# zkp-gravity/0g-halo2

Measured on AMD Instinct MI355X. Metric: create_proof proofs/hour, model_28input_256entry_1hash_1bpi, higher is better.
Workload: dtype u32x8 (254-bit Montgomery integers)

## Files before the change

### 0g-halo2_amd/csrc/common.h

```cpp
#pragma once

#include <hip/hip_runtime.h>
#include <hip/hip_ext.h>

#include <array>
#include <atomic>
#include <cstdarg>
#include <cstdio>
#include <cstring>
#include <map>
#include <mutex>
#include <string>
#include <vector>

#include "../../include/zg_halo2.h"
#include "curve.h"

namespace zg {

void set_error(const char* fmt, ...);

#define ZG_HIP(call)                                                                         \
    do {                                                                                     \
        hipError_t _e = (call);                                                              \
// ... 16 lines not shown

#define ZG_REQUIRE(cond, status, ...)   \
    do {                                \
        if (!(cond)) {                  \
            ::zg::set_error(__VA_ARGS__); \
            return (status);            \
        }                               \
    } while (0)

static_assert(sizeof(Fe) == 32 && sizeof(zg_fr) == 32, "field element layout");
static_assert(sizeof(Affine) == 64 && sizeof(zg_g1_affine) == 64, "affine layout");
static_assert(sizeof(Jac) == 96 && sizeof(zg_g1) == 96, "jacobian layout");
static_assert(sizeof(XYZZ) == 128, "xyzz layout");

struct WsBlock {
    void* p = nullptr;
    size_t cap = 0;
    bool used = false;
};

struct TwiddleKey {
    uint32_t log_n;
    std::array<uint64_t, 4> omega;
    bool operator<(const TwiddleKey& o) const {
        if (log_n != o.log_n) return log_n < o.log_n;
        return omega < o.omega;
    }
};

}

namespace zg {
struct DeviceState {
    std::mutex mu;
    std::map<TwiddleKey, Fe*> twiddles;
    int refs = 0;
    bool msm_attrs = false, ntt_attrs = false;
};
DeviceState& device_state(int device);
}

struct zg_ctx {
    int device = 0;
    hipStream_t stream = nullptr;
    int num_cus = 256;
    std::vector<zg::WsBlock> pool;
    void* pinned = nullptr;
    size_t pinned_cap = 0;
    std::recursive_mutex mu;
// ... 60 lines not shown
            failed = true;
            return nullptr;
        }
        held.push_back(p);
        return reinterpret_cast<T*>(p);
    }
};
int pinned_reserve(zg_ctx* ctx, size_t bytes);
void gate_yield(zg_ctx* ctx);
uint32_t tuning_generation();

zg_ctx::ProfRec* prof_slot(zg_ctx* ctx, const char* name, double algo_bytes, double unit_bytes);
#define ZG_LAUNCH_U(ctx, name, bytes, unit, kernel, grid, block, lds, ...)                               \
    do {                                                                                                 \
        zg_ctx::ProfRec* _zg_r = (ctx)->profiling ? ::zg::prof_slot((ctx), (name), (double)(bytes), (double)(unit)) : nullptr; \
        if (_zg_r)                                                                                       \
            hipExtLaunchKernelGGL(kernel, grid, block, lds, (ctx)->stream, _zg_r->e0, _zg_r->e1, 0, __VA_ARGS__); \
        else                                                                                             \
            hipLaunchKernelGGL(kernel, grid, block, lds, (ctx)->stream, __VA_ARGS__);                    \
    } while (0)
#define ZG_LAUNCH(ctx, name, bytes, kernel, grid, block, lds, ...) \
    ZG_LAUNCH_U(ctx, name, bytes, 0.0, kernel, grid, block, lds, __VA_ARGS__)

int get_twiddles(zg_ctx* ctx, uint32_t log_n, const Fe& omega, Fe** out);

Fe host_domain_omega(uint32_t log_n);

enum Knob : int {
    K_MSM_C,
    K_MSM_K,
    K_MSM_K_LAT,
    K_MSM_RB,
    K_MSM_LANES,
    K_MSM_STRIP,
    K_MSM_NAF,
    K_MSM_NAF_GL,
    K_MSM_RUNS,
    K_EVALH_GROUPED,
    K_EVALH9,
    K_SPLIT_DOMAIN,
    K_LAT_SPLIT_K,
    K_LAT_FULL_C,
    K_LAT_FULL_K,
    K_LAZY_DOT,
    K_MSM_AFFINE,
    K_MSM_HEAVY,
    K_LAT_PULL,
// ... 11 lines not shown
```

### 0g-halo2_amd/csrc/field9.h

```cpp
#pragma once

#include "curve.h"
#include "field.h"

namespace zg {

struct F9 {
    int32_t l[9];
};

constexpr int32_t MASK29 = (1 << 29) - 1;

struct Fq9Params {
    static __device__ __forceinline__ int32_t p(int i) {
        constexpr int32_t P[9] = {0x187cfd47, 0x010460b6, 0x1c72a34f, 0x02d522d0, 0x1585d978,
                                  0x02db40c0, 0x00a6e141, 0x0e5c2634, 0x0030644e};
        return P[i];
    }
    static constexpr uint32_t INV29 = 0x04866389u;
    static __device__ __forceinline__ F9 one() {
        return F9{{0x157ccc21, 0x141c2758, 0x185230d3, 0x014c0419, 0x0aa36fb9, 0x1d4240ce, 0x11d54c07, 0x052ac7a8, 0x000dc836}};
    }
    static __device__ __forceinline__ F9 k256() {
        return F9{{0x058f0d9d, 0x1aea1c6e, 0x11c2cf74, 0x11d651eb, 0x1462c0a7, 0x11b7bc3c, 0x1cbd99ba, 0x183340fb, 0x000e0a77}};
// ... 363 lines not shown
            inf = true;
            return;
        }
        const F9 u = f9_norm(f9_add(qy, qy));
        const F9 v = Fq9::sqr(u);
        const F9 w = Fq9::mul(u, v);
        const F9 s = Fq9::mul(qx, v);
        const F9 x2 = Fq9::sqr(qx);
        const F9 m = f9_norm(f9_add(f9_add(x2, x2), x2));
        a.x = f9_norm(f9_sub(f9_sub(Fq9::sqr(m), s), s));
        a.y = f9_norm(f9_sub(Fq9::mul(m, f9_norm(f9_sub(s, a.x))), Fq9::mul(w, f9_norm(qy))));
        a.zz = v;
        a.zzz = w;
        return;
    }
    const F9 ppp = Fq9::mul(p, pp);
    const F9 qq = Fq9::mul(a.x, pp);
    const F9 x3 = f9_norm(f9_sub(f9_sub(f9_sub(Fq9::sqr(r), ppp), qq), qq));
    const F9 t = f9_sub(qq, x3);
    a.y = Fq9::mul2<true>(r, t, a.y, ppp);
    a.x = x3;
    a.zz = Fq9::mul(a.zz, pp);
    a.zzz = Fq9::mul(a.zzz, ppp);
}

__device__ __noinline__ XYZZ9 xyzz9_dbl(const XYZZ9& a) {
    if (xyzz9_is_identity(a)) return a;
    XYZZ9 o;
    const F9 u = f9_norm(f9_add(a.y, a.y));
    const F9 v = Fq9::sqr(u);
    const F9 w = Fq9::mul(u, v);
    const F9 s = Fq9::mul(a.x, v);
    const F9 xx = Fq9::sqr(a.x);
    const F9 m = f9_norm(f9_add(f9_add(xx, xx), xx));
    o.x = f9_norm(f9_sub(f9_sub(Fq9::sqr(m), s), s));
    o.y = f9_norm(f9_sub(Fq9::mul(m, f9_norm(f9_sub(s, o.x))), Fq9::mul(w, a.y)));
    o.zz = Fq9::mul(v, a.zz);
    o.zzz = Fq9::mul(w, a.zzz);
    return o;
}

__device__ __forceinline__ XYZZ9 xyzz9_add(const XYZZ9& a, const XYZZ9& b) {
    if (xyzz9_is_identity(a)) return b;
    if (xyzz9_is_identity(b)) return a;
    const F9 u1 = Fq9::mul(a.x, b.zz);
    const F9 u2 = Fq9::mul(b.x, a.zz);
// ... 254 lines not shown
```

### 0g-halo2_amd/csrc/msm.hip

```cpp
#include <cstdlib>

#include "msm.h"
#include "field9.h"

namespace zg {

constexpr uint32_t MSM_K_THROUGHPUT = 48, MSM_K_LATENCY = 16;
constexpr uint32_t MSM_MAX_C = 16;
constexpr uint32_t MSM_LEN_BINS = 128;
constexpr uint32_t MSM_HEAVY = 16;
constexpr uint32_t MSM_HEAVY_THROUGHPUT = 4;
constexpr uint32_t MSM_AFFINE_ROUNDS = 0;
constexpr uint32_t MSM_MAX_BATCH = 4096;

__device__ __forceinline__ Fe ld_fe_g(const Fe* p) {
    Fe r;
    const uint4* q = reinterpret_cast<const uint4*>(p);
    uint4 a = q[0], b = q[1];
    r.l[0] = a.x; r.l[1] = a.y; r.l[2] = a.z; r.l[3] = a.w;
    r.l[4] = b.x; r.l[5] = b.y; r.l[6] = b.z; r.l[7] = b.w;
    return r;
}
__device__ __forceinline__ void st_fe_g(Fe* p, const Fe& v) {
    uint4* q = reinterpret_cast<uint4*>(p);
// ... 567 lines not shown
        }
    };
    scan(true);
    const F9 before = t ? sh[t - 1] : Fq9Params::one();
    if (t == AFF_TOP - 1) {
        const Fe inv8 = Fq::inv(f9_reduce_pack<Fq9Params>(sh[t]));
        tinv = Fq9::mul(f9_unpack(inv8), Fq9Params::k271());
    }
    __syncthreads();
    scan(false);
    const F9 after = t + 1 < AFF_TOP ? sh[t + 1] : Fq9Params::one();
    F9 u = Fq9::mul(Fq9::mul(tinv, before), after);
    if (t >= n2) return;
    size_t e = t + ((n2 - 1 - t) / AFF_TOP) * AFF_TOP;
#pragma unroll 1
    for (;; e -= AFF_TOP) {
        const F9 v = ld_f9_soa(val2, n2, e);
        st_f9_soa(val2, n2, e, Fq9::mul(u, ld_f9_soa(pfx2, n2, e)));
        u = Fq9::mul(u, v);
        if (e < AFF_TOP) break;
    }
}

template <bool PAIR, bool AFF = false>
__global__ __launch_bounds__(256) void msm_accumulate_kernel(
    const Affine* __restrict__ table_a, const Affine* __restrict__ table_b, uint32_t split, uint32_t n_table,
    uint32_t c, uint32_t windows, uint32_t n,
    const uint32_t* __restrict__ tot, const uint32_t* __restrict__ toff, const uint32_t* __restrict__ ttotal,
    const uint32_t* __restrict__ sorted, uint32_t max_tasks, XYZZ9* __restrict__ partial,
    const Affine* __restrict__ run_a, const Affine* __restrict__ run_b, uint64_t run_mask, uint32_t per,
    const uint32_t* __restrict__ stoff, const uint32_t* __restrict__ sbucket, size_t cap, uint32_t R,
    const Affine* __restrict__ pts) {
    const uint32_t lane = blockIdx.x * blockDim.x + threadIdx.x;
    const uint32_t t = PAIR ? lane >> 1 : lane;
    const bool role_a = !PAIR || (lane & 1u) == 0;
    uint32_t b = blockIdx.y;
    if (t >= ttotal[b]) return;
    const uint32_t vj = b % per;
    const bool runs = vj < 64 && ((run_mask >> vj) & 1ull);
    const Affine* table = vj < split ? (runs ? run_a : table_a) : (runs ? run_b : table_b);
    const uint32_t nb = 1u << (c - 1);
    const uint32_t* to = toff + (size_t)b * (nb + 2);
    const uint32_t* sto = stoff + (size_t)b * (nb + 2);
    uint32_t lo = 0, hi = nb + 1;
    while (hi - lo > 1) {
        uint32_t mid = (lo + hi) >> 1;
        if (sto[mid] <= t) lo = mid;
        else hi = mid;
    }
    const uint32_t k = sbucket[(size_t)b * (nb + 1) + lo];
    const uint32_t j = t - sto[lo];
    const uint32_t first = tot[(size_t)b * (nb + 2) + k] >> R;
    const uint32_t total = (tot[(size_t)b * (nb + 2) + k + 1] >> R) - first;
    const uint32_t nt = to[k + 1] - to[k];
    const uint32_t share = total / nt, extra = total % nt;
    const uint32_t start = first + j * share + (j < extra ? j : extra);
    const uint32_t len = share + (j < extra ? 1u : 0u);
    const uint32_t* so = sorted + (size_t)b * cap + start;
    XYZZ9* dst = partial + (size_t)b * max_tasks + to[k] + j;
    bool inf = true;
    if constexpr (PAIR) {
        PairAcc acc;
        for (uint32_t e = 0; e < len; e++) {
            uint32_t ent = so[e];
            uint32_t i = ent & 0x7fffffu, w = (ent >> 23) & 0xffu;
            const Affine* src = table + (size_t)w * n_table + i;
            const F9 qx = f9_unpack(ld_fe_g(&src->x));
            F9 qy = f9_unpack(ld_fe_g(&src->y));
            if (f9_limbs_zero(qx) && f9_limbs_zero(qy)) continue;
            if (ent >> 31) qy = f9_neg(qy);
            xmadd_pair(acc, inf, qx, qy, role_a);
        }
        if (inf) {
            if (role_a) st_xyzz9(dst, xyzz9_identity());
        } else if (role_a) {
            st_f9(&dst->x, acc.m);
            st_f9(&dst->zz, acc.z);
        } else {
            st_f9(&dst->y, acc.m);
            st_f9(&dst->zzz, acc.z);
        }
    } else if constexpr (AFF) {
        XYZZ9 acc;
        const Affine* src = pts + (size_t)b * (cap >> R) + start;
        for (uint32_t e = 0; e < len; e++) {
            const F9 qx = f9_unpack(ld_fe_g(&src[e].x));
            const F9 qy = f9_unpack(ld_fe_g(&src[e].y));
            if (f9_limbs_zero(qx) && f9_limbs_zero(qy)) continue;
            xyzz9_madd(acc, inf, qx, qy);
        }
        st_xyzz9(dst, inf ? xyzz9_identity() : acc);
    } else {
        XYZZ9 acc;
        for (uint32_t e = 0; e < len; e++) {
            uint32_t ent = so[e];
            uint32_t i = ent & 0x7fffffu, w = (ent >> 23) & 0xffu;
            const Affine* src = table + (size_t)w * n_table + i;
            const F9 qx = f9_unpack(ld_fe_g(&src->x));
            F9 qy = f9_unpack(ld_fe_g(&src->y));
            if (f9_limbs_zero(qx) && f9_limbs_zero(qy)) continue;
            if (ent >> 31) qy = f9_neg(qy);
            xyzz9_madd(acc, inf, qx, qy);
        }
        st_xyzz9(dst, inf ? xyzz9_identity() : acc);
    }
}

constexpr uint32_t MSM_RB = 256;


constexpr uint32_t MSM_HEAVY_WGS = 256;
template <int L>
__global__ __launch_bounds__(256 * L) void msm_heavy_kernel(const XYZZ9* __restrict__ partial,
                                                                     const uint32_t* __restrict__ toff,
                                                                     const uint32_t* __restrict__ hlist,
                                                                     const uint32_t* __restrict__ nheavy, uint32_t max_tasks,
                                                                     uint32_t max_heavy, uint32_t c,
                                                                     XYZZ9* __restrict__ hsum, uint32_t B) {
    __shared__ XYZZ9 sh[256];
    __shared__ uint32_t nh_of[MSM_MAX_BATCH];
    const uint32_t nb = 1u << (c - 1);
    const uint32_t j = threadIdx.x / L, role = threadIdx.x % L;
    int any = 0;
    for (uint32_t b = threadIdx.x; b < B; b += blockDim.x) {
        uint32_t v = nheavy[b];
        if (v > max_heavy) v = max_heavy;
        nh_of[b] = v;
// ... 1204 lines not shown
```

### 0g-halo2_amd/csrc/ntt.hip

```cpp
#include "poly.h"
#include "field9.h"

namespace zg {

struct NttArgs {
    const Fe* in;
    Fe* out;
    const Fe* tw;
    const Fe* tw_m;
    uint32_t tw_shift;
    size_t in_stride;
    size_t out_stride;
    uint32_t in_per, out_per;
    size_t in_outer, out_outer;
    uint32_t log_n, log_n1, log_n2;
    uint32_t in_len;
    uint32_t out_len;
    uint32_t coset_in;
    uint32_t coset_out;
    uint32_t scale_out;
    Fe zin0, zin1, zin2, zout1, zout2, scale;
};

__device__ __forceinline__ uint32_t bitrev(uint32_t v, uint32_t bits) {
    return bits == 0 ? 0u : (__brev(v) >> (32 - bits));
}

__device__ __forceinline__ Fe ld_fe(const Fe* p) {
    Fe r;
    const uint4* q = reinterpret_cast<const uint4*>(p);
    uint4 a = q[0], b = q[1];
    r.l[0] = a.x; r.l[1] = a.y; r.l[2] = a.z; r.l[3] = a.w;
    r.l[4] = b.x; r.l[5] = b.y; r.l[6] = b.z; r.l[7] = b.w;
    return r;
}

__device__ __forceinline__ void st_fe(Fe* p, const Fe& v) {
    uint4* q = reinterpret_cast<uint4*>(p);
    q[0] = make_uint4(v.l[0], v.l[1], v.l[2], v.l[3]);
    q[1] = make_uint4(v.l[4], v.l[5], v.l[6], v.l[7]);
}

template <int LOG_T, bool COLS, bool FIRST>
__global__ __launch_bounds__(1 << (LOG_T - 2)) void ntt_pass_kernel(NttArgs a) {
// ... 43 lines not shown
            const Fe w = ld_fe(a.tw + ((size_t)t << tw_shift));
            const uint32_t s = slot(t);
            TL[s] = make_uint4(w.l[0], w.l[1], w.l[2], w.l[3]);
            TH[s] = make_uint4(w.l[4], w.l[5], w.l[6], w.l[7]);
        }
    }

    for (uint32_t e = tid; e < tile; e += NT) {
        uint32_t g, li;
        if (COLS) {
            uint32_t c = e & (cnt - 1), j1 = e >> log_cnt;
            g = j1 * N2 + base + c;
            li = e;
        } else {
            uint32_t j2 = e & (M - 1), r = e >> log_m;
            g = (base + r) * N2 + j2;
            li = e;
        }
        Fe v;
        if (FIRST) {
            if (g < a.in_len) {
                v = ld_fe(in + g);
                if (a.coset_in) {
                    uint32_t m3 = g % 3u;
                    if (m3 == 1) v = Fr::mul(v, a.zin1);
                    else if (m3 == 2) v = Fr::mul(v, a.zin2);
                    else if (a.coset_in == 2) v = Fr::mul(v, a.zin0);
                }
            } else {
                v = fe_zero();
            }
        } else {
            v = ld_fe(in + g);
        }
        stx(li, v);
    }
    __syncthreads();

    auto at = [&](uint32_t sub, uint32_t e) { return COLS ? (e << log_cnt) + sub : (sub << log_m) + e; };
    uint32_t st = 0;
    if (FIRST && COLS && log_m >= 2) {
        const uint32_t nz_rows = (a.in_len + N2 - 1) >> a.log_n2;
        const uint32_t quarter = M >> 2, half = M >> 1;
        if (nz_rows <= quarter) {
            for (uint32_t g = tid; g < tile / 4; g += NT) {
                const uint32_t sub = g & (cnt - 1), i = g >> log_cnt;
                if (i >= nz_rows) continue;
                const uint32_t i0 = at(sub, i), i1 = at(sub, i + quarter), i2 = at(sub, i + half), i3 = at(sub, i + half + quarter);
                const Fe x0 = ldx(i0);
                Fe a2 = x0;
// ... 59 lines not shown
            } else {
                b = bf & (M / 2 - 1);
                s = bf >> (log_m - 1);
            }
            uint32_t blk = b >> log_half, i = b & (half - 1);
            uint32_t lo = (blk << (log_half + 1)) + i, hi = lo + half;
            uint32_t ilo = at(s, lo), ihi = at(s, hi);
            Fe u = ldx(ilo), v = ldx(ihi);
            stx(ilo, Fr::add(u, v));
            Fe d = Fr::sub(u, v);
            uint32_t twi = i << st;
            if (twi != 0) d = Fr::mul(d, ldt(twi));
            stx(ihi, d);
        }
        __syncthreads();
    }

    if (COLS) {
        for (uint32_t e = tid; e < tile; e += NT) {
            uint32_t c = e & (cnt - 1), pos = e >> log_cnt;
            uint32_t k1 = bitrev(pos, log_m);
            uint32_t j2 = base + c;
            Fe v = ldx(e);
            uint32_t ti = j2 * k1;
            if (ti != 0) v = Fr::mul(v, ld_fe(a.tw + ti));
            st_fe(out + (size_t)k1 * N2 + j2, v);
        }
    } else {
        for (uint32_t e = tid; e < tile; e += NT) {
            uint32_t r = e & (cnt - 1), k2 = e >> log_cnt;
            uint32_t pos = bitrev(k2, log_m);
            uint32_t k = (base + r) + N1 * k2;
            if (k >= a.out_len) continue;
            Fe v = ldx((r << log_m) + pos);
            if (a.scale_out) v = Fr::mul(v, a.scale);
            if (a.coset_out) {
                uint32_t m3 = k % 3u;
                if (m3 == 1) v = Fr::mul(v, a.zout1);
                else if (m3 == 2) v = Fr::mul(v, a.zout2);
            }
            st_fe(out + k, v);
        }
    }
}

template <int LOG_T, bool COLS, bool FIRST>
__global__ __launch_bounds__(1 << (LOG_T - 2)) void ntt9_pass_kernel(NttArgs a) {
    constexpr uint32_t T = 1u << LOG_T;
    constexpr uint32_t NT = T / 4;
    extern __shared__ __align__(16) unsigned char smem[];
    const uint32_t log_m = COLS ? a.log_n1 : a.log_n2;
    const uint32_t M = 1u << log_m;
    const uint32_t S = a.tw_shift;
    const uint32_t TWN = (M / 2) >> S ? (M / 2) >> S : 1;
    uint4* XL = reinterpret_cast<uint4*>(smem);
    uint4* XH = XL + T;
    uint4* TL = XH + T;
    uint4* TH = TL + TWN;
    int32_t* X8 = reinterpret_cast<int32_t*>(TH + TWN);
    int32_t* T8 = X8 + T;
    auto slot = [](uint32_t i) { return i ^ ((i >> 3) & 7u) ^ ((i >> 6) & 7u) ^ ((i >> 9) & 7u); };
    auto ld3 = [&](const uint4* L, const uint4* H, const int32_t* E, uint32_t i) {
// ... 9 lines not shown
        const uint32_t s = slot(i);
        L[s] = make_uint4((uint32_t)v.l[0], (uint32_t)v.l[1], (uint32_t)v.l[2], (uint32_t)v.l[3]);
        H[s] = make_uint4((uint32_t)v.l[4], (uint32_t)v.l[5], (uint32_t)v.l[6], (uint32_t)v.l[7]);
        E[s] = v.l[8];
    };
    auto ldx = [&](uint32_t i) { return ld3(XL, XH, X8, i); };
    auto stx = [&](uint32_t i, const F9& v) { st3(XL, XH, X8, i, v); };
    const Fe* twm9 = a.tw_m + M;
    auto ldt = [&](uint32_t i, uint32_t st) { return st >= S ? ld3(TL, TH, T8, i >> S) : f9_unpack(ld_fe(twm9 + i)); };

    const uint32_t tid = threadIdx.x;
    const uint32_t N1 = 1u << a.log_n1, N2 = 1u << a.log_n2;
    uint32_t log_cnt = LOG_T - log_m;
    if (!COLS && log_cnt > a.log_n1) log_cnt = a.log_n1;
    const uint32_t cnt = 1u << log_cnt;
    const uint32_t tile = M << log_cnt;

    uint32_t nblk = gridDim.x, bid = blockIdx.x;
    if ((nblk & 7u) == 0) bid = (bid & 7u) * (nblk >> 3) + (bid >> 3);
    const uint32_t base = bid << log_cnt;

    const Fe* in = a.in + (size_t)(blockIdx.y / a.in_per) * a.in_outer + (size_t)(blockIdx.y % a.in_per) * a.in_stride;
    Fe* out = a.out + (size_t)(blockIdx.y / a.out_per) * a.out_outer + (size_t)(blockIdx.y % a.out_per) * a.out_stride;
    const Fe* tw9 = a.tw + ((size_t)1 << a.log_n);

    for (uint32_t t = tid; t < (M / 2) >> S; t += NT) st3(TL, TH, T8, t, f9_unpack(ld_fe(twm9 + (t << S))));
    for (uint32_t e = tid; e < tile; e += NT) {
        uint32_t g;
        if (COLS) {
            uint32_t c = e & (cnt - 1), j1 = e >> log_cnt;
            g = j1 * N2 + base + c;
        } else {
            uint32_t j2 = e & (M - 1), r = e >> log_m;
            g = (base + r) * N2 + j2;
        }
        F9 v;
        if (FIRST) {
            if (g < a.in_len) {
                v = f9_unpack(ld_fe(in + g));
                if (a.coset_in) {
                    uint32_t m3 = g % 3u;
                    if (m3 == 1) v = Fr9::mul(v, f9_unpack(a.zin1));
                    else if (m3 == 2) v = Fr9::mul(v, f9_unpack(a.zin2));
                    else if (a.coset_in == 2) v = Fr9::mul(v, f9_unpack(a.zin0));
                }
            } else {
#pragma unroll
                for (int i = 0; i < 9; i++) v.l[i] = 0;
            }
        } else {
            v = f9_unpack(ld_fe(in + g));
        }
        stx(e, v);
    }
    __syncthreads();

    auto at = [&](uint32_t sub, uint32_t e) { return COLS ? (e << log_cnt) + sub : (sub << log_m) + e; };
    uint32_t st = 0, grp = 0;
    if (FIRST && COLS && log_m >= 2) {
        const uint32_t nz_rows = (a.in_len + N2 - 1) >> a.log_n2;
        const uint32_t quarter = M >> 2, half = M >> 1;
        if (nz_rows <= quarter) {
            for (uint32_t g = tid; g < tile / 4; g += NT) {
                const uint32_t sub = g & (cnt - 1), i = g >> log_cnt;
                if (i >= nz_rows) continue;
                const uint32_t i0 = at(sub, i), i1 = at(sub, i + quarter), i2 = at(sub, i + half), i3 = at(sub, i + half + quarter);
                const F9 x0 = ldx(i0);
// ... 51 lines not shown
    for (; st < log_m; st++) {
        for (uint32_t bf = tid; bf < nbf; bf += NT) {
            uint32_t s, b;
            if (COLS) {
                s = bf & (cnt - 1);
                b = bf >> log_cnt;
            } else {
                b = bf & (M / 2 - 1);
                s = bf >> (log_m - 1);
            }
            const uint32_t ilo = at(s, b << 1), ihi = at(s, (b << 1) + 1);
            const F9 u = ldx(ilo), v = ldx(ihi);
            stx(ilo, f9_norm(f9_add(u, v)));
            stx(ihi, f9_norm(f9_sub(u, v)));
        }
        __syncthreads();
    }

    if (COLS) {
        for (uint32_t e = tid; e < tile; e += NT) {
            uint32_t c = e & (cnt - 1), pos = e >> log_cnt;
            uint32_t k1 = bitrev(pos, log_m);
            uint32_t j2 = base + c;
            const F9 v = Fr9::mul(ldx(e), f9_unpack(ld_fe(tw9 + j2 * k1)));
            st_fe(out + (size_t)k1 * N2 + j2, f9_reduce_pack<Fr9Params>(v));
        }
    } else {
        for (uint32_t e = tid; e < tile; e += NT) {
            uint32_t r = e & (cnt - 1), k2 = e >> log_cnt;
            uint32_t pos = bitrev(k2, log_m);
            uint32_t k = (base + r) + N1 * k2;
            if (k >= a.out_len) continue;
            F9 v = ldx((r << log_m) + pos);
            if (a.scale_out) v = Fr9::mul(v, f9_unpack(a.scale));
            if (a.coset_out) {
                uint32_t m3 = k % 3u;
                if (m3 == 1) v = Fr9::mul(v, f9_unpack(a.zout1));
                else if (m3 == 2) v = Fr9::mul(v, f9_unpack(a.zout2));
            }
            st_fe(out + k, f9_reduce_pack<Fr9Params>(v));
        }
    }
}

__global__ void twiddle_kernel(Fe* tw, Fe omega, uint32_t n) {
    constexpr uint32_t CH = 16;
    uint32_t i0 = (blockIdx.x * blockDim.x + threadIdx.x) * CH;
    if (i0 >= n) return;
    const Fe c261 = Fr9Params::c261_fe();
    Fe cur = Fr::pow_u64(omega, i0);
    for (uint32_t j = 0; j < CH && i0 + j < n; j++) {
        st_fe(tw + i0 + j, cur);
        st_fe(tw + n + i0 + j, Fr::mul(cur, c261));
        cur = Fr::mul(cur, omega);
    }
}

int get_twiddles(zg_ctx* ctx, uint32_t log_n, const Fe& omega, Fe** out) {
    TwiddleKey key;
    key.log_n = log_n;
    memcpy(key.omega.data(), &omega, 32);
    DeviceState& ds = device_state(ctx->device);
    std::lock_guard<std::mutex> lock(ds.mu);
    auto it = ds.twiddles.find(key);
    if (it != ds.twiddles.end()) {
        *out = it->second;
        return ZG_OK;
    }
    uint32_t n = 1u << log_n;
    Fe* tw = nullptr;
    gate_yield(ctx);
    ZG_HIP(hipMalloc(&tw, (size_t)2 * n * sizeof(Fe)));
    uint32_t threads = 256, per = 16;
    uint32_t blocks = (n + threads * per - 1) / (threads * per);
    hipLaunchKernelGGL(twiddle_kernel, dim3(blocks), dim3(threads), 0, ctx->stream, tw, omega, n);
    hipError_t e = hipGetLastError();
    if (e == hipSuccess) e = hipStreamSynchronize(ctx->stream);
    if (e != hipSuccess) {
        (void)hipFree(tw);
        set_error("get_twiddles: %s", hipGetErrorString(e));
        return ZG_ERR_HIP;
    }
    ds.twiddles[key] = tw;
    *out = tw;
    return ZG_OK;
}

struct NttPlan {
    const Fe* in;
    size_t in_stride;
    Fe* out;
    size_t out_stride;
    size_t batch;
    uint32_t log_n;
    Fe omega;
    uint32_t in_len, out_len;
    Grouping grp;
    uint32_t coset_in = 0;
    bool coset_out = false, scale_out = false;
    Fe zin0, zin1, zin2, zout1, zout2, scale;
};

static int sub_twiddles(zg_ctx* ctx, const NttPlan& p, uint32_t log_m, uint32_t log_t, const Fe** table, uint32_t* shift) {
    Fe om = p.omega;
    for (uint32_t i = log_m; i < p.log_n; i++) om = Fr::sqr(om);
    Fe* t = nullptr;
    ZG_TRY(get_twiddles(ctx, log_m, om, &t));
    *table = t;
    const uint32_t room = log_t == 10 ? 113u : 227u;
    uint32_t s = 0;
    while ((((1u << log_m) / 2) >> s) > room) s++;
    *shift = s;
    return ZG_OK;
}
static size_t nine_lds_bytes(uint32_t T, uint32_t log_m, uint32_t shift) {
    const uint32_t twn = ((1u << log_m) / 2) >> shift;
    return (size_t)(T + (twn ? twn : 1)) * 36;
}

template <int LOG_T, bool NINE>
static int launch_passes(zg_ctx* ctx, const NttPlan& p, const Fe* tw, Fe* tmp, size_t tmp_stride) {
    constexpr uint32_t T = 1u << LOG_T;
    constexpr size_t ELEM = NINE ? 36 : sizeof(Fe);
    NttArgs a;
    memset(&a, 0, sizeof(a));
    a.tw = tw;
    a.log_n = p.log_n;
    a.in_len = p.in_len;
    a.out_len = p.out_len;
    a.coset_in = p.coset_in;
    a.coset_out = p.coset_out;
    a.scale_out = p.scale_out;
    a.zin0 = p.zin0; a.zin1 = p.zin1; a.zin2 = p.zin2; a.zout1 = p.zout1; a.zout2 = p.zout2; a.scale = p.scale;
    if (NINE) {
        const Fe c261 = Fr9Params::c261_fe();
        for (Fe* c : {&a.zin0, &a.zin1, &a.zin2, &a.zout1, &a.zout2, &a.scale}) *c = Fr::mul(*c, c261);
    }
    const uint32_t N = 1u << p.log_n;
    const uint32_t gper = p.grp.per ? p.grp.per : 0xffffffffu;
    const double pass_bytes = (double)p.batch * ((double)p.in_len + (double)p.out_len) * 32.0;
    const double unit_bytes = ctx->unit_next >= 0.0 ? ctx->unit_next : pass_bytes;
    ctx->unit_next = -1.0;
    const double pts = (double)p.batch * (double)(1u << p.log_n) * 32.0;
    dim3 block(T / 4);
    const bool single = p.log_n <= (uint32_t)LOG_T;
    if (single) {
        a.log_n1 = 0;
        a.log_n2 = p.log_n;
        a.in = p.in; a.in_stride = p.in_stride;
        a.out = p.out; a.out_stride = p.out_stride;
        a.in_per = a.out_per = gper; a.in_outer = p.grp.in_outer; a.out_outer = p.grp.out_outer;
        size_t lds = (size_t)(T + (N > 1 ? N / 2 : 1)) * ELEM;
        if (NINE) {
            ZG_TRY(sub_twiddles(ctx, p, a.log_n2, LOG_T, &a.tw_m, &a.tw_shift));
            lds = nine_lds_bytes(T, a.log_n2, a.tw_shift);
        }
        if (NINE)
            ZG_LAUNCH_U(ctx, "ntt_single", pass_bytes, unit_bytes, (ntt9_pass_kernel<LOG_T, false, true>), dim3(1, (uint32_t)p.batch), block, lds, a);
        else
// ... 29 lines not shown
        a.in_per = 0xffffffffu; a.in_outer = 0;
        a.out_per = gper; a.out_outer = p.grp.out_outer;
        uint32_t cnt = T / N2;
        if (cnt > N1) cnt = N1;
        size_t lds = (size_t)(T + (N2 > 1 ? N2 / 2 : 1)) * ELEM;
        if (NINE) {
            ZG_TRY(sub_twiddles(ctx, p, a.log_n2, LOG_T, &a.tw_m, &a.tw_shift));
            lds = nine_lds_bytes(T, a.log_n2, a.tw_shift);
        }
        if (NINE)
            ZG_LAUNCH_U(ctx, "ntt_rows", pts + (double)p.batch * (double)p.out_len * 32.0, unit_bytes, (ntt9_pass_kernel<LOG_T, false, false>),
                        dim3(N1 / cnt, (uint32_t)p.batch), block, lds, a);
        else
            ZG_LAUNCH_U(ctx, "ntt_rows", pts + (double)p.batch * (double)p.out_len * 32.0, unit_bytes, (ntt_pass_kernel<LOG_T, false, false>),
                        dim3(N1 / cnt, (uint32_t)p.batch), block, lds, a);
        ZG_HIP(hipGetLastError());
    }
    return ZG_OK;
}

static uint32_t ntt_log_t(uint32_t log_n) { return log_n <= 16 ? 10u : 11u; }
bool ntt_needs_tmp(uint32_t log_n) { return log_n > ntt_log_t(log_n); }

int ntt_run(zg_ctx* ctx, const NttPlan& p, Fe* tmp, size_t tmp_stride) {
    ZG_REQUIRE(p.log_n <= 22, ZG_ERR_UNSUPPORTED, "ntt: log_n %u > 22 not built", p.log_n);
    if (p.batch == 0) return ZG_OK;
    Fe* tw = nullptr;
    ZG_TRY(get_twiddles(ctx, p.log_n, p.omega, &tw));
    const int k9 = knob(K_NTT9);
    const bool nine = k9 < 0 ? ctx->msm_pair : k9 != 0;
    if (ntt_log_t(p.log_n) == 10) return nine ? launch_passes<10, true>(ctx, p, tw, tmp, tmp_stride) : launch_passes<10, false>(ctx, p, tw, tmp, tmp_stride);
    return nine ? launch_passes<11, true>(ctx, p, tw, tmp, tmp_stride) : launch_passes<11, false>(ctx, p, tw, tmp, tmp_stride);
}

static int ensure_lds_attr(zg_ctx* ctx) {
    DeviceState& ds = device_state(ctx->device);
    std::lock_guard<std::mutex> lock(ds.mu);
    if (ds.ntt_attrs) return ZG_OK;
    const int big = 160 * 1024;
    ZG_HIP(hipFuncSetAttribute((const void*)ntt_pass_kernel<11, true, true>,
                               hipFuncAttributeMaxDynamicSharedMemorySize, big));
    ZG_HIP(hipFuncSetAttribute((const void*)ntt_pass_kernel<11, false, true>,
                               hipFuncAttributeMaxDynamicSharedMemorySize, big));
    ZG_HIP(hipFuncSetAttribute((const void*)ntt_pass_kernel<11, false, false>,
                               hipFuncAttributeMaxDynamicSharedMemorySize, big));
    ZG_HIP(hipFuncSetAttribute((const void*)ntt_pass_kernel<10, true, true>,
                               hipFuncAttributeMaxDynamicSharedMemorySize, big));
    ZG_HIP(hipFuncSetAttribute((const void*)ntt_pass_kernel<10, false, true>,
                               hipFuncAttributeMaxDynamicSharedMemorySize, big));
    ZG_HIP(hipFuncSetAttribute((const void*)ntt_pass_kernel<10, false, false>,
                               hipFuncAttributeMaxDynamicSharedMemorySize, big));
    ZG_HIP(hipFuncSetAttribute((const void*)ntt9_pass_kernel<11, true, true>, hipFuncAttributeMaxDynamicSharedMemorySize, big));
    ZG_HIP(hipFuncSetAttribute((const void*)ntt9_pass_kernel<11, false, true>, hipFuncAttributeMaxDynamicSharedMemorySize, big));
    ZG_HIP(hipFuncSetAttribute((const void*)ntt9_pass_kernel<11, false, false>, hipFuncAttributeMaxDynamicSharedMemorySize, big));
    ZG_HIP(hipFuncSetAttribute((const void*)ntt9_pass_kernel<10, true, true>, hipFuncAttributeMaxDynamicSharedMemorySize, big));
// ... 37 lines not shown
int coeff_to_extended_dev(zg_ctx* ctx, const Fe* d_in, size_t in_stride, Fe* d_out, size_t out_stride,
                          size_t batch, uint32_t k, uint32_t ext_k, bool hat) {
    return coeff_to_coset_dev(ctx, d_in, in_stride, 1u << k, d_out, out_stride, batch, ext_k, hat, ctx->coset_gen, nullptr);
}

int coeff_to_coset_dev(zg_ctx* ctx, const Fe* d_in, size_t in_stride, uint32_t in_len, Fe* d_out, size_t out_stride,
                       size_t batch, uint32_t ext_k, bool hat, const Fe& shift, const Grouping* grp) {
    ZG_REQUIRE(in_len <= (1u << ext_k), ZG_ERR_INVALID_ARG, "coeff_to_coset: %u coefficients for 2^%u points", in_len, ext_k);
    ZG_TRY(ensure_lds_attr(ctx));
    WsScope ws(ctx);
    NttPlan p;
    if (grp) p.grp = *grp;
    p.in = d_in; p.in_stride = in_stride;
    p.out = d_out; p.out_stride = out_stride;
    p.batch = batch;
    p.log_n = ext_k;
    p.omega = host_domain_omega(ext_k);
    p.in_len = in_len;
    p.out_len = 1u << ext_k;
    p.coset_in = 1;
    p.zin0 = Fr::one();
    p.zin1 = shift;
    p.zin2 = Fr::sqr(shift);
    if (hat) {
        const Fe c32 = Fr::from_u64(32);
        p.coset_in = 2;
        p.zin0 = c32;
        p.zin1 = Fr::mul(p.zin1, c32);
        p.zin2 = Fr::mul(p.zin2, c32);
    }
    size_t n = (size_t)1 << ext_k;
    Fe* tmp = nullptr;
    if (ntt_needs_tmp(ext_k)) {
        tmp = ws.get<Fe>(batch * n);
        if (!tmp) return ZG_ERR_OOM;
    } else if (d_in == d_out) {
    }
    return ntt_run(ctx, p, tmp, n);
}

int extended_to_coeff_dev(zg_ctx* ctx, Fe* d_evals, uint32_t k, uint32_t ext_k, size_t out_len,
                          Fe* d_out, bool unhat) {
    (void)k;
    return coset_to_coeff_dev(ctx, d_evals, ext_k, out_len, d_out, unhat, ctx->coset_gen, 1, 0, 0);
}

int coset_to_coeff_dev(zg_ctx* ctx, Fe* d_evals, uint32_t ext_k, size_t out_len, Fe* d_out, bool unhat, const Fe& shift,
                       size_t batch, size_t in_stride, size_t out_stride) {
    ZG_TRY(ensure_lds_attr(ctx));
    WsScope ws(ctx);
    size_t n = (size_t)1 << ext_k;
    ZG_REQUIRE(out_len <= n, ZG_ERR_INVALID_ARG, "extended_to_coeff: out_len %zu > 2^%u", out_len, ext_k);
    NttPlan p;
    p.in = d_evals; p.in_stride = in_stride ? in_stride : n;
    p.out = d_out; p.out_stride = out_stride ? out_stride : out_len;
    p.batch = batch;
    p.log_n = ext_k;
    p.omega = Fr::inv(host_domain_omega(ext_k));
    p.in_len = (uint32_t)n;
    p.out_len = (uint32_t)out_len;
    p.scale_out = true;
    p.scale = Fr::inv(Fr::from_u64((uint64_t)n * (unhat ? 32u : 1u)));
    p.coset_out = true;
    p.zout1 = Fr::sqr(shift);
    p.zout2 = shift;
    Fe* tmp = nullptr;
    if (ntt_needs_tmp(ext_k)) {
        tmp = ws.get<Fe>(batch * n);
        if (!tmp) return ZG_ERR_OOM;
    } else if (d_out != d_evals) {
    }
    return ntt_run(ctx, p, tmp, n);
}

}

using namespace zg;

extern "C" {

int zg_ntt_batch_dev(zg_ctx* ctx, void* d_a, size_t stride_elems, size_t batch, uint32_t log_n,
                     const zg_fr* omega, const zg_fr* divisor) {
    ZG_REQUIRE(ctx && d_a && omega, ZG_ERR_INVALID_ARG, "zg_ntt_batch_dev: null argument");
    ZG_REQUIRE(stride_elems >= ((size_t)1 << log_n) || batch <= 1, ZG_ERR_INVALID_ARG,
               "zg_ntt_batch_dev: stride %zu < 2^%u", stride_elems, log_n);
    ZG_ENTER(ctx);
// ... 96 lines not shown
```

### 0g-halo2_amd/csrc/poly.hip

```cpp
#include "poly.h"
#include "poly_eval.h"
#include "field9.h"

namespace zg {

__host__ __device__ __forceinline__ uint32_t rotl32(uint32_t x, int sft) { return (x << sft) | (x >> (32 - sft)); }
#define ZG_QR(a, b, c, d)                       \
    do {                                        \
        a += b; d ^= a; d = rotl32(d, 16);      \
        c += d; b ^= c; b = rotl32(b, 12);      \
        a += b; d ^= a; d = rotl32(d, 8);       \
        c += d; b ^= c; b = rotl32(b, 7);       \
    } while (0)

__host__ __device__ inline Fe rand_fr(const uint32_t* key, uint32_t tag, uint64_t index) {
    Fe v;
    for (uint32_t attempt = 0;; attempt++) {
        uint32_t x0 = 0x61707865u, x1 = 0x3320646eu, x2 = 0x79622d32u, x3 = 0x6b206574u;
        uint32_t x4 = key[0], x5 = key[1], x6 = key[2], x7 = key[3], x8 = key[4], x9 = key[5], x10 = key[6], x11 = key[7];
        uint32_t x12 = attempt, x13 = tag, x14 = (uint32_t)index, x15 = (uint32_t)(index >> 32);
        for (int r = 0; r < 10; r++) {
            ZG_QR(x0, x4, x8, x12);
            ZG_QR(x1, x5, x9, x13);
            ZG_QR(x2, x6, x10, x14);
// ... 81 lines not shown
                          uint32_t n, uint32_t tag, Fe* base, size_t base_bs, size_t col_stride, uint32_t ncols,
                          uint32_t row0, uint32_t nrows, uint32_t blind_tag) {
    const uint32_t total = n + ncols * nrows;
    if (nb == 0) return ZG_OK;
    ZG_LAUNCH(ctx, "random_poly", (double)nb * n * 32, random_and_blind_kernel, dim3((total + 255) / 256, nb), dim3(256), 0, pc,
              out, out_bs, out2, out2_bs, n, tag, base, base_bs, col_stride, ncols, row0, nrows, blind_tag);
    ZG_HIP(hipGetLastError());
    return ZG_OK;
}

__global__ __launch_bounds__(256) void lookup_compress_kernel(DevCircuit c, Cols cols_all, const ProofConst* __restrict__ pc,
                                                              Fe* cin, Fe* ctab, uint32_t n, Fe* raw_in, Fe* raw_tab,
                                                              uint32_t usable) {
    uint32_t row = blockIdx.x * blockDim.x + threadIdx.x;
    const uint32_t b = blockIdx.z;
    uint32_t l = blockIdx.y;
    if (row >= n) return;
    const Cols cols = cols_of(cols_all, b);
    const Fe theta = pc[b].theta;
    const DLookup* lk = c.lookups + l;
    l += b * c.n_lookups;
    Fe ai = fe_zero(), ti = fe_zero();
    for (uint32_t e = 0; e < lk->width; e++) {
        ai = Fr::add(Fr::mul(ai, theta), eval_poly(c, cols, lk->inputs[e], row));
        ti = Fr::add(Fr::mul(ti, theta), eval_poly(c, cols, lk->tables[e], row));
    }
    stg(cin + (size_t)l * n + row, ai);
    stg(ctab + (size_t)l * n + row, ti);
    if (raw_in) {
        Fe ra, rt;
        if (row < usable) {
            ra = Fr::to_raw(ai);
            rt = Fr::to_raw(ti);
        } else {
#pragma unroll
            for (int j = 0; j < 8; j++) ra.l[j] = rt.l[j] = 0xffffffffu;
        }
        stg(raw_in + (size_t)l * n + row, ra);
        stg(raw_tab + (size_t)l * n + row, rt);
    }
}

int poly_lookup_compress(zg_ctx* ctx, const DevCircuit& c, const Cols& cols, const ProofConst* pc, uint32_t nb, Fe* cin,
                         Fe* ctab, uint32_t n, Fe* raw_in, Fe* raw_tab, uint32_t usable) {
    if (c.n_lookups == 0 || nb == 0) return ZG_OK;
    ZG_LAUNCH(ctx, "lookup_compress", (double)nb * c.n_lookups * n * 64, lookup_compress_kernel,
              dim3((n + 255) / 256, c.n_lookups, nb), dim3(256), 0, c, cols, pc, cin, ctab, n, raw_in, raw_tab, usable);
    ZG_HIP(hipGetLastError());
// ... 500 lines not shown
        }
        Fe current_delta = Fr::mul(pr.pc->eh_delta_start[a.zpow - 1], ldg(a.ext_tw + idx));
        for (uint32_t s = 0; s < c.n_sets; s++) {
            uint32_t c0 = s * c.chunk, c1 = c0 + c.chunk;
            if (c1 > c.n_perm) c1 = c.n_perm;
            Fe left = ldg(pr.pz_cos + (size_t)s * en + r_next);
            Fe right = ldg(pr.pz_cos + (size_t)s * en + idx);
            for (uint32_t col = c0; col < c1; col++) {
                const zg_query q = c.perm_cols[col];
                const Fe* base = q.kind == ZG_FIXED ? pr.cols.fixed : q.kind == ZG_ADVICE ? pr.cols.advice : pr.cols.instance;
                Fe v = ldg(base + ((size_t)q.column << a.cols.log_size) + idx);
                Fe sg = ldg(a.sigma_cos + (size_t)col * en + idx);
                left = Fr::mul(left, Fr::add(Fr::add(Fr::mul(beta, sg), v), gamma));
                right = Fr::mul(right, Fr::add(Fr::add(v, current_delta), gamma));
                current_delta = Fr::mul(current_delta, a.delta);
            }
            value = Fr::add(Fr::mul(value, y), Fr::mul(Fr::sub(left, right), lactive));
        }
    }
    for (uint32_t l = 0; l < c.n_lookups; l++) {
        const DLookup* lk = c.lookups + l;
        Fe ai = fe_zero(), ti = fe_zero();
        for (uint32_t e = 0; e < lk->width; e++) {
            ai = Fr::add(Fr::mul(ai, theta), eval_poly(c, pr.cols, lk->inputs[e], idx));
            ti = Fr::add(Fr::mul(ti, theta), eval_poly(c, pr.cols, lk->tables[e], idx));
        }
        const Fe* zc = pr.lz_cos + (size_t)l * en;
        const Fe* ap = pr.pin_cos + (size_t)l * a.perm_stride;
        const Fe* sp = pr.ptab_cos + (size_t)l * a.perm_stride;
        const Fe z = ldg(zc + idx), apv = ldg(ap + idx), spv = ldg(sp + idx);
        value = Fr::add(Fr::mul(value, y), Fr::mul(Fr::sub(Fr::one(), z), l0));
        value = Fr::add(Fr::mul(value, y), Fr::mul(Fr::sub(Fr::sqr(z), z), llast));
        Fe lft = Fr::mul(Fr::mul(Fr::add(apv, beta), Fr::add(spv, gamma)), ldg(zc + r_next));
        Fe rgt = Fr::mul(Fr::mul(Fr::add(ai, beta), Fr::add(ti, gamma)), z);
        value = Fr::add(Fr::mul(value, y), Fr::mul(Fr::sub(lft, rgt), lactive));
        Fe ams = Fr::sub(apv, spv);
        value = Fr::add(Fr::mul(value, y), Fr::mul(ams, l0));
        value = Fr::add(Fr::mul(value, y), Fr::mul(Fr::mul(ams, Fr::sub(apv, ldg(ap + r_prev))), lactive));
    }
    value = Fr::mul(value, ldg(a.t_eval + (idx & a.t_mask)));
    stg(pr.h + idx, value);
}


__device__ __forceinline__ F9 ld9(const Fe* p) { return f9_unpack(ldg(p)); }

__device__ __forceinline__ F9 eval_poly9(const DevCircuit& c, const DMono* monos, const Cols& cols, zg_poly p, uint32_t row) {
    const uint32_t mask = (1u << cols.log_size) - 1u;
// ... 907 lines not shown
```

Measured before the change: 5.153 million.

## Fold NTT scaling into twiddles, chain affine MSM adds, skip first theta multiply

Folds the inverse-NTT output scale and the hat factor into a scaled twiddle table, or into the coset constants, so the separate per-element multiplies go away. Also drops the zero-index twiddle branch. The MSM accumulate kernel now starts each bucket chain with an affine pair-add instead of a mixed add onto identity. Lookup compression skips the multiply by theta on the first term. In exchange the code caches extra scaled twiddle tables, capped per size, which costs device memory and a one-time generation cost.

```diff
diff --git a/0g-halo2_amd/csrc/common.h b/0g-halo2_amd/csrc/common.h
--- a/0g-halo2_amd/csrc/common.h
+++ b/0g-halo2_amd/csrc/common.h
@@ -62,9 +62,11 @@
 struct TwiddleKey {
     uint32_t log_n;
     std::array<uint64_t, 4> omega;
+    std::array<uint64_t, 4> scale;
     bool operator<(const TwiddleKey& o) const {
         if (log_n != o.log_n) return log_n < o.log_n;
-        return omega < o.omega;
+        if (omega != o.omega) return omega < o.omega;
+        return scale < o.scale;
     }
 };
 
@@ -171,7 +173,7 @@
 #define ZG_LAUNCH(ctx, name, bytes, kernel, grid, block, lds, ...) \
     ZG_LAUNCH_U(ctx, name, bytes, 0.0, kernel, grid, block, lds, __VA_ARGS__)
 
-int get_twiddles(zg_ctx* ctx, uint32_t log_n, const Fe& omega, Fe** out);
+int get_twiddles(zg_ctx* ctx, uint32_t log_n, const Fe& omega, Fe** out, const Fe* scale = nullptr);
 
 Fe host_domain_omega(uint32_t log_n);
 
diff --git a/0g-halo2_amd/csrc/field9.h b/0g-halo2_amd/csrc/field9.h
--- a/0g-halo2_amd/csrc/field9.h
+++ b/0g-halo2_amd/csrc/field9.h
@@ -409,6 +409,40 @@
     a.x = x3;
     a.zz = Fq9::mul(a.zz, pp);
     a.zzz = Fq9::mul(a.zzz, ppp);
+}
+
+__device__ __forceinline__ void xyzz9_from_pair(const F9& x1, const F9& y1, const F9& x2, const F9& y2, XYZZ9& out, bool& inf) {
+    const F9 p = f9_sub(x2, x1);
+    const F9 r = f9_sub(f9_norm(y2), y1);
+    const F9 pp = Fq9::sqr(p);
+    if (__builtin_expect(pp.l[8] >= 0 && Fq9::is_zero_mod_p(pp), 0)) {
+        const F9 rr = Fq9::sqr(r);
+        if (!Fq9::is_zero_mod_p(rr)) {
+            inf = true;
+            return;
+        }
+        const F9 u = f9_norm(f9_add(y1, y1));
+        const F9 v = Fq9::sqr(u);
+        const F9 w = Fq9::mul(u, v);
+        const F9 s = Fq9::mul(x1, v);
+        const F9 xx = Fq9::sqr(x1);
+        const F9 m = f9_norm(f9_add(f9_add(xx, xx), xx));
+        const F9 x3 = f9_norm(f9_sub(f9_sub(Fq9::sqr(m), s), s));
+        out.y = f9_norm(f9_sub(Fq9::mul(m, f9_norm(f9_sub(s, x3))), Fq9::mul(w, y1)));
+        out.x = x3;
+        out.zz = v;
+        out.zzz = w;
+        inf = false;
+        return;
+    }
+    const F9 ppp = Fq9::mul(p, pp);
+    const F9 qq = Fq9::mul(x1, pp);
+    const F9 x3 = f9_norm(f9_sub(f9_sub(f9_sub(Fq9::sqr(r), ppp), qq), qq));
+    out.y = Fq9::mul2<true>(r, f9_sub(qq, x3), y1, ppp);
+    out.x = x3;
+    out.zz = pp;
+    out.zzz = ppp;
+    inf = false;
 }
 
 __device__ __noinline__ XYZZ9 xyzz9_dbl(const XYZZ9& a) {
diff --git a/0g-halo2_amd/csrc/msm.hip b/0g-halo2_amd/csrc/msm.hip
--- a/0g-halo2_amd/csrc/msm.hip
+++ b/0g-halo2_amd/csrc/msm.hip
@@ -613,6 +613,24 @@
     }
 }
 
+__device__ __forceinline__ void chain_madd(XYZZ9& acc, bool& inf, bool& aff, const F9& qx, const F9& qy) {
+    if (inf) {
+        acc.x = qx;
+        acc.y = f9_norm(qy);
+        inf = false;
+        aff = true;
+    } else if (aff) {
+        aff = false;
+        xyzz9_from_pair(acc.x, acc.y, qx, qy, acc, inf);
+    } else {
+        xyzz9_madd(acc, inf, qx, qy);
+    }
+}
+__device__ __forceinline__ void chain_store(XYZZ9* dst, XYZZ9& acc, bool inf, bool aff) {
+    if (aff) acc.zz = acc.zzz = Fq9Params::one();
+    st_xyzz9(dst, inf ? xyzz9_identity() : acc);
+}
+
 template <bool PAIR, bool AFF = false>
 __global__ __launch_bounds__(256) void msm_accumulate_kernel(
     const Affine* __restrict__ table_a, const Affine* __restrict__ table_b, uint32_t split, uint32_t n_table,
@@ -649,7 +667,7 @@
     const uint32_t len = share + (j < extra ? 1u : 0u);
     const uint32_t* so = sorted + (size_t)b * cap + start;
     XYZZ9* dst = partial + (size_t)b * max_tasks + to[k] + j;
-    bool inf = true;
+    bool inf = true, aff = false;
     if constexpr (PAIR) {
         PairAcc acc;
         for (uint32_t e = 0; e < len; e++) {
@@ -678,9 +696,9 @@
             const F9 qx = f9_unpack(ld_fe_g(&src[e].x));
             const F9 qy = f9_unpack(ld_fe_g(&src[e].y));
             if (f9_limbs_zero(qx) && f9_limbs_zero(qy)) continue;
-            xyzz9_madd(acc, inf, qx, qy);
-        }
-        st_xyzz9(dst, inf ? xyzz9_identity() : acc);
+            chain_madd(acc, inf, aff, qx, qy);
+        }
+        chain_store(dst, acc, inf, aff);
     } else {
         XYZZ9 acc;
         for (uint32_t e = 0; e < len; e++) {
@@ -691,9 +709,9 @@
             F9 qy = f9_unpack(ld_fe_g(&src->y));
             if (f9_limbs_zero(qx) && f9_limbs_zero(qy)) continue;
             if (ent >> 31) qy = f9_neg(qy);
-            xyzz9_madd(acc, inf, qx, qy);
-        }
-        st_xyzz9(dst, inf ? xyzz9_identity() : acc);
+            chain_madd(acc, inf, aff, qx, qy);
+        }
+        chain_store(dst, acc, inf, aff);
     }
 }
 
diff --git a/0g-halo2_amd/csrc/ntt.hip b/0g-halo2_amd/csrc/ntt.hip
--- a/0g-halo2_amd/csrc/ntt.hip
+++ b/0g-halo2_amd/csrc/ntt.hip
@@ -7,6 +7,7 @@
     const Fe* in;
     Fe* out;
     const Fe* tw;
+    const Fe* tw_x;
     const Fe* tw_m;
     uint32_t tw_shift;
     size_t in_stride;
@@ -19,7 +20,7 @@
     uint32_t coset_in;
     uint32_t coset_out;
     uint32_t scale_out;
-    Fe zin0, zin1, zin2, zout1, zout2, scale;
+    Fe zin0, zin1, zin2, zout0, zout1, zout2, scale;
 };
 
 __device__ __forceinline__ uint32_t bitrev(uint32_t v, uint32_t bits) {
@@ -109,10 +110,8 @@
             if (g < a.in_len) {
                 v = ld_fe(in + g);
                 if (a.coset_in) {
-                    uint32_t m3 = g % 3u;
-                    if (m3 == 1) v = Fr::mul(v, a.zin1);
-                    else if (m3 == 2) v = Fr::mul(v, a.zin2);
-                    else if (a.coset_in == 2) v = Fr::mul(v, a.zin0);
+                    const uint32_t m3 = g % 3u;
+                    if (m3 != 0 || a.coset_in == 2) v = Fr::mul(v, m3 == 1 ? a.zin1 : m3 == 2 ? a.zin2 : a.zin0);
                 }
             } else {
                 v = fe_zero();
@@ -218,8 +217,7 @@
             uint32_t k1 = bitrev(pos, log_m);
             uint32_t j2 = base + c;
             Fe v = ldx(e);
-            uint32_t ti = j2 * k1;
-            if (ti != 0) v = Fr::mul(v, ld_fe(a.tw + ti));
+            v = Fr::mul(v, ld_fe(a.tw_x + j2 * k1));
             st_fe(out + (size_t)k1 * N2 + j2, v);
         }
     } else {
@@ -231,9 +229,8 @@
             Fe v = ldx((r << log_m) + pos);
             if (a.scale_out) v = Fr::mul(v, a.scale);
             if (a.coset_out) {
-                uint32_t m3 = k % 3u;
-                if (m3 == 1) v = Fr::mul(v, a.zout1);
-                else if (m3 == 2) v = Fr::mul(v, a.zout2);
+                const uint32_t m3 = k % 3u;
+                if (m3 != 0 || a.coset_out == 2) v = Fr::mul(v, m3 == 1 ? a.zout1 : m3 == 2 ? a.zout2 : a.zout0);
             }
             st_fe(out + k, v);
         }
@@ -289,7 +286,6 @@
 
     const Fe* in = a.in + (size_t)(blockIdx.y / a.in_per) * a.in_outer + (size_t)(blockIdx.y % a.in_per) * a.in_stride;
     Fe* out = a.out + (size_t)(blockIdx.y / a.out_per) * a.out_outer + (size_t)(blockIdx.y % a.out_per) * a.out_stride;
-    const Fe* tw9 = a.tw + ((size_t)1 << a.log_n);
 
     for (uint32_t t = tid; t < (M / 2) >> S; t += NT) st3(TL, TH, T8, t, f9_unpack(ld_fe(twm9 + (t << S))));
     for (uint32_t e = tid; e < tile; e += NT) {
@@ -306,10 +302,8 @@
             if (g < a.in_len) {
                 v = f9_unpack(ld_fe(in + g));
                 if (a.coset_in) {
-                    uint32_t m3 = g % 3u;
-                    if (m3 == 1) v = Fr9::mul(v, f9_unpack(a.zin1));
-                    else if (m3 == 2) v = Fr9::mul(v, f9_unpack(a.zin2));
-                    else if (a.coset_in == 2) v = Fr9::mul(v, f9_unpack(a.zin0));
+                    const uint32_t m3 = g % 3u;
+                    if (m3 != 0 || a.coset_in == 2) v = Fr9::mul(v, f9_unpack(m3 == 1 ? a.zin1 : m3 == 2 ? a.zin2 : a.zin0));
                 }
             } else {
 #pragma unroll
@@ -407,7 +401,7 @@
             uint32_t c = e & (cnt - 1), pos = e >> log_cnt;
             uint32_t k1 = bitrev(pos, log_m);
             uint32_t j2 = base + c;
-            const F9 v = Fr9::mul(ldx(e), f9_unpack(ld_fe(tw9 + j2 * k1)));
+            const F9 v = Fr9::mul(ldx(e), f9_unpack(ld_fe(a.tw_x + j2 * k1)));
             st_fe(out + (size_t)k1 * N2 + j2, f9_reduce_pack<Fr9Params>(v));
         }
     } else {
@@ -419,21 +413,20 @@
             F9 v = ldx((r << log_m) + pos);
             if (a.scale_out) v = Fr9::mul(v, f9_unpack(a.scale));
             if (a.coset_out) {
-                uint32_t m3 = k % 3u;
-                if (m3 == 1) v = Fr9::mul(v, f9_unpack(a.zout1));
-                else if (m3 == 2) v = Fr9::mul(v, f9_unpack(a.zout2));
+                const uint32_t m3 = k % 3u;
+                if (m3 != 0 || a.coset_out == 2) v = Fr9::mul(v, f9_unpack(m3 == 1 ? a.zout1 : m3 == 2 ? a.zout2 : a.zout0));
             }
             st_fe(out + k, f9_reduce_pack<Fr9Params>(v));
         }
     }
 }
 
-__global__ void twiddle_kernel(Fe* tw, Fe omega, uint32_t n) {
+__global__ void twiddle_kernel(Fe* tw, Fe omega, Fe s, uint32_t n) {
     constexpr uint32_t CH = 16;
     uint32_t i0 = (blockIdx.x * blockDim.x + threadIdx.x) * CH;
     if (i0 >= n) return;
     const Fe c261 = Fr9Params::c261_fe();
-    Fe cur = Fr::pow_u64(omega, i0);
+    Fe cur = Fr::mul(Fr::pow_u64(omega, i0), s);
     for (uint32_t j = 0; j < CH && i0 + j < n; j++) {
         st_fe(tw + i0 + j, cur);
         st_fe(tw + n + i0 + j, Fr::mul(cur, c261));
@@ -441,10 +434,13 @@
     }
 }
 
-int get_twiddles(zg_ctx* ctx, uint32_t log_n, const Fe& omega, Fe** out) {
+constexpr uint32_t MAX_SCALED_TABLES = 8;
+int get_twiddles(zg_ctx* ctx, uint32_t log_n, const Fe& omega, Fe** out, const Fe* scale) {
+    const Fe s = scale ? *scale : Fr::one();
     TwiddleKey key;
     key.log_n = log_n;
     memcpy(key.omega.data(), &omega, 32);
+    memcpy(key.scale.data(), &s, 32);
     DeviceState& ds = device_state(ctx->device);
     std::lock_guard<std::mutex> lock(ds.mu);
     auto it = ds.twiddles.find(key);
@@ -452,13 +448,22 @@
         *out = it->second;
         return ZG_OK;
     }
+    if (scale) {
+        const Fe one = Fr::one();
+        uint32_t scaled = 0;
+        for (const auto& kv : ds.twiddles) scaled += kv.first.log_n == log_n && memcmp(kv.first.scale.data(), &one, 32) != 0;
+        if (scaled >= MAX_SCALED_TABLES) {
+            *out = nullptr;
+            return ZG_OK;
+        }
+    }
     uint32_t n = 1u << log_n;
     Fe* tw = nullptr;
     gate_yield(ctx);
     ZG_HIP(hipMalloc(&tw, (size_t)2 * n * sizeof(Fe)));
     uint32_t threads = 256, per = 16;
     uint32_t blocks = (n + threads * per - 1) / (threads * per);
-    hipLaunchKernelGGL(twiddle_kernel, dim3(blocks), dim3(threads), 0, ctx->stream, tw, omega, n);
+    hipLaunchKernelGGL(twiddle_kernel, dim3(blocks), dim3(threads), 0, ctx->stream, tw, omega, s, n);
     hipError_t e = hipGetLastError();
     if (e == hipSuccess) e = hipStreamSynchronize(ctx->stream);
     if (e != hipSuccess) {
@@ -482,8 +487,10 @@
     uint32_t in_len, out_len;
     Grouping grp;
     uint32_t coset_in = 0;
-    bool coset_out = false, scale_out = false;
-    Fe zin0, zin1, zin2, zout1, zout2, scale;
+    uint32_t coset_out = 0;
+    bool scale_out = false;
+    bool hat = false;
+    Fe zin0, zin1, zin2, zout0, zout1, zout2, scale;
 };
 
 static int sub_twiddles(zg_ctx* ctx, const NttPlan& p, uint32_t log_m, uint32_t log_t, const Fe** table, uint32_t* shift) {
@@ -504,22 +511,23 @@
 }
 
 template <int LOG_T, bool NINE>
-static int launch_passes(zg_ctx* ctx, const NttPlan& p, const Fe* tw, Fe* tmp, size_t tmp_stride) {
+static int launch_passes(zg_ctx* ctx, const NttPlan& p, const Fe* tw, const Fe* tw_x, Fe* tmp, size_t tmp_stride) {
     constexpr uint32_t T = 1u << LOG_T;
     constexpr size_t ELEM = NINE ? 36 : sizeof(Fe);
     NttArgs a;
     memset(&a, 0, sizeof(a));
     a.tw = tw;
+    a.tw_x = tw_x;
     a.log_n = p.log_n;
     a.in_len = p.in_len;
     a.out_len = p.out_len;
     a.coset_in = p.coset_in;
     a.coset_out = p.coset_out;
     a.scale_out = p.scale_out;
-    a.zin0 = p.zin0; a.zin1 = p.zin1; a.zin2 = p.zin2; a.zout1 = p.zout1; a.zout2 = p.zout2; a.scale = p.scale;
+    a.zin0 = p.zin0; a.zin1 = p.zin1; a.zin2 = p.zin2; a.zout0 = p.zout0; a.zout1 = p.zout1; a.zout2 = p.zout2; a.scale = p.scale;
     if (NINE) {
         const Fe c261 = Fr9Params::c261_fe();
-        for (Fe* c : {&a.zin0, &a.zin1, &a.zin2, &a.zout1, &a.zout2, &a.scale}) *c = Fr::mul(*c, c261);
+        for (Fe* c : {&a.zin0, &a.zin1, &a.zin2, &a.zout0, &a.zout1, &a.zout2, &a.scale}) *c = Fr::mul(*c, c261);
     }
     const uint32_t N = 1u << p.log_n;
     const uint32_t gper = p.grp.per ? p.grp.per : 0xffffffffu;
@@ -595,15 +603,56 @@
 static uint32_t ntt_log_t(uint32_t log_n) { return log_n <= 16 ? 10u : 11u; }
 bool ntt_needs_tmp(uint32_t log_n) { return log_n > ntt_log_t(log_n); }
 
-int ntt_run(zg_ctx* ctx, const NttPlan& p, Fe* tmp, size_t tmp_stride) {
-    ZG_REQUIRE(p.log_n <= 22, ZG_ERR_UNSUPPORTED, "ntt: log_n %u > 22 not built", p.log_n);
-    if (p.batch == 0) return ZG_OK;
+int ntt_run(zg_ctx* ctx, const NttPlan& plan, Fe* tmp, size_t tmp_stride) {
+    ZG_REQUIRE(plan.log_n <= 22, ZG_ERR_UNSUPPORTED, "ntt: log_n %u > 22 not built", plan.log_n);
+    if (plan.batch == 0) return ZG_OK;
+    NttPlan p = plan;
     Fe* tw = nullptr;
     ZG_TRY(get_twiddles(ctx, p.log_n, p.omega, &tw));
     const int k9 = knob(K_NTT9);
     const bool nine = k9 < 0 ? ctx->msm_pair : k9 != 0;
-    if (ntt_log_t(p.log_n) == 10) return nine ? launch_passes<10, true>(ctx, p, tw, tmp, tmp_stride) : launch_passes<10, false>(ctx, p, tw, tmp, tmp_stride);
-    return nine ? launch_passes<11, true>(ctx, p, tw, tmp, tmp_stride) : launch_passes<11, false>(ctx, p, tw, tmp, tmp_stride);
+    const Fe c32 = Fr::from_u64(32);
+    const size_t half = (size_t)1 << p.log_n;
+    const Fe c261 = Fr9Params::c261_fe();
+    ZG_REQUIRE(memcmp(&c261, &c32, sizeof(Fe)) == 0, ZG_ERR_UNSUPPORTED, "ntt: 2^261 mod r is not the field element 32");
+    const Fe* tw_x = tw + (nine ? half : 0);
+    bool rides = false;
+    if (ntt_needs_tmp(p.log_n) && (p.scale_out || p.hat)) {
+        if (!nine && !p.scale_out) {
+            tw_x = tw + half;
+            rides = true;
+        } else {
+            Fe s = p.scale_out ? p.scale : Fr::one();
+            if (p.hat) s = Fr::mul(s, c32);
+            Fe* tws = nullptr;
+            ZG_TRY(get_twiddles(ctx, p.log_n, p.omega, &tws, &s));
+            if (tws) {
+                tw_x = tws + (nine ? half : 0);
+                rides = true;
+            }
+        }
+    }
+    if (rides) {
+        p.scale_out = false;
+    } else {
+        if (p.hat) {
+            ZG_REQUIRE(p.coset_in == 1, ZG_ERR_UNSUPPORTED, "ntt: a hat transform without coset constants");
+            p.coset_in = 2;
+            p.zin0 = c32;
+            p.zin1 = Fr::mul(p.zin1, c32);
+            p.zin2 = Fr::mul(p.zin2, c32);
+        }
+        if (p.scale_out && p.coset_out == 1) {
+            p.coset_out = 2;
+            p.zout0 = p.scale;
+            p.zout1 = Fr::mul(p.zout1, p.scale);
+            p.zout2 = Fr::mul(p.zout2, p.scale);
+            p.scale_out = false;
+        }
+    }
+    if (ntt_log_t(p.log_n) == 10)
+        return nine ? launch_passes<10, true>(ctx, p, tw, tw_x, tmp, tmp_stride) : launch_passes<10, false>(ctx, p, tw, tw_x, tmp, tmp_stride);
+    return nine ? launch_passes<11, true>(ctx, p, tw, tw_x, tmp, tmp_stride) : launch_passes<11, false>(ctx, p, tw, tw_x, tmp, tmp_stride);
 }
 
 static int ensure_lds_attr(zg_ctx* ctx) {
@@ -687,13 +736,7 @@
     p.zin0 = Fr::one();
     p.zin1 = shift;
     p.zin2 = Fr::sqr(shift);
-    if (hat) {
-        const Fe c32 = Fr::from_u64(32);
-        p.coset_in = 2;
-        p.zin0 = c32;
-        p.zin1 = Fr::mul(p.zin1, c32);
-        p.zin2 = Fr::mul(p.zin2, c32);
-    }
+    p.hat = hat;
     size_t n = (size_t)1 << ext_k;
     Fe* tmp = nullptr;
     if (ntt_needs_tmp(ext_k)) {
@@ -726,7 +769,7 @@
     p.out_len = (uint32_t)out_len;
     p.scale_out = true;
     p.scale = Fr::inv(Fr::from_u64((uint64_t)n * (unhat ? 32u : 1u)));
-    p.coset_out = true;
+    p.coset_out = 1;
     p.zout1 = Fr::sqr(shift);
     p.zout2 = shift;
     Fe* tmp = nullptr;
diff --git a/0g-halo2_amd/csrc/poly.hip b/0g-halo2_amd/csrc/poly.hip
--- a/0g-halo2_amd/csrc/poly.hip
+++ b/0g-halo2_amd/csrc/poly.hip
@@ -127,8 +127,9 @@
     l += b * c.n_lookups;
     Fe ai = fe_zero(), ti = fe_zero();
     for (uint32_t e = 0; e < lk->width; e++) {
-        ai = Fr::add(Fr::mul(ai, theta), eval_poly(c, cols, lk->inputs[e], row));
-        ti = Fr::add(Fr::mul(ti, theta), eval_poly(c, cols, lk->tables[e], row));
+        const Fe in = eval_poly(c, cols, lk->inputs[e], row), tb = eval_poly(c, cols, lk->tables[e], row);
+        ai = e ? Fr::add(Fr::mul(ai, theta), in) : in;
+        ti = e ? Fr::add(Fr::mul(ti, theta), tb) : tb;
     }
     stg(cin + (size_t)l * n + row, ai);
     stg(ctab + (size_t)l * n + row, ti);
@@ -675,8 +676,9 @@
         const DLookup* lk = c.lookups + l;
         Fe ai = fe_zero(), ti = fe_zero();
         for (uint32_t e = 0; e < lk->width; e++) {
-            ai = Fr::add(Fr::mul(ai, theta), eval_poly(c, pr.cols, lk->inputs[e], idx));
-            ti = Fr::add(Fr::mul(ti, theta), eval_poly(c, pr.cols, lk->tables[e], idx));
+            const Fe in = eval_poly(c, pr.cols, lk->inputs[e], idx), tb = eval_poly(c, pr.cols, lk->tables[e], idx);
+            ai = e ? Fr::add(Fr::mul(ai, theta), in) : in;
+            ti = e ? Fr::add(Fr::mul(ti, theta), tb) : tb;
         }
         const Fe* zc = pr.lz_cos + (size_t)l * en;
         const Fe* ap = pr.pin_cos + (size_t)l * a.perm_stride;
```

Measured after the change: 5.277 million, median of 6. +2.4%, better.
